# AechPro/rlgym-ppo

Hardware: AMD Instinct MI355X
Metric: ppo_update_samples_per_sec (higher is better)
Workload: dtype f32; 1 GPU; configs[1]: 4096 agents x 128 steps = 524,288-sample buffer, obs 107 f32, 90 discrete actions, 256x3 policy + critic; batch 524,288, minibatch 65,536

## Files before the change

rlgym_ppo_amd/csrc/api.hip:

```cpp
#include "build_id.h"
#include <math.h>
#include <stdarg.h>
#include <string.h>

#include "common.hpp"

namespace rlppo {

static thread_local char g_err[512] = "";

void set_error(const char *fmt, ...) {
    va_list ap;
    va_start(ap, fmt);
    vsnprintf(g_err, sizeof(g_err), fmt, ap);
    va_end(ap);
}

static int64_t padded_width(int64_t d) {
    const int64_t p16 = round_up(d, 16), p64 = round_up(d, 64);
    return (p64 - p16) * 10 >= p64 ? p16 : p64;
}
static int64_t padded_out(int64_t d) {
    if (d <= 32) return 32;
    if (d <= 64) return 64;
// ... 583 lines not shown
        RLPPO_HIP(hipEventCreateWithFlags(&b.ev_join[s], hipEventDisableTiming));
        RLPPO_HIP(hipEventCreateWithFlags(&b.ev_slot[s], hipEventDisableTiming));
        RLPPO_HIP(hipEventCreateWithFlags(&b.ev_mid[s], hipEventDisableTiming));
    }
    return 0;
}
static int order_after(hipStream_t to, hipStream_t from, hipEvent_t ev) {
    RLPPO_HIP(hipEventRecord(ev, from));
    RLPPO_HIP(hipStreamWaitEvent(to, ev, 0));
    return 0;
}

static size_t tn_layer_floats(const NetLayout &net, int l, int64_t mb, int prec) {
    size_t f = tn_partial_floats(net.L[l].out, net.L[l].in, mb);
    if (net.L[l].out == 1) {
        const size_t g = (size_t)cdiv(mb, 64) * (size_t)(net.L[l].pin + 4);
        if (g > f) f = g;
    }
    if (prec == 1 && l == net.n_layers - 1) {
        const size_t g = thin_dw_ws_floats(net.L[l].out, net.L[l].pin, mb);
        if (g > f) f = g;
    }
    return (f + 3) / 4 * 4;
}
static size_t tn_ws_floats(const NetLayout &net, int64_t mb, int prec) {
    size_t m = 0;
    for (int l = 0; l < net.n_layers; ++l) {
        const size_t f = tn_layer_floats(net, l, mb, prec);
        m = f > m ? f : m;
    }
    return m;
}
static int g_group_dw = 1;
struct DwList {
    TnProduct p[2 * RLPPO_MAX_LAYERS];
    int n = 0;
    void add(const LayerLayout &L, const float *dY, const RowSource &X, float *grad) {
        TnProduct &q = p[n++];
        q.dY = dY; q.ldy = L.pout; q.ny_valid = L.pout; q.X = X.x; q.ldx = X.ld; q.kx_valid = L.pin;
        q.dW = grad + L.off_flat_w; q.db = grad + L.off_flat_b; q.out = L.out; q.in = L.in;
        q.rowtab = X.rowtab; q.src_rows = X.src_rows;
    }
};
static bool dw_is_gemv(const NetLayout &net, int l) { return l == net.n_layers - 1 && l > 0 && gemv_head_ok(net.L[l].out, net.L[l].pin); }
static size_t tn_region_floats(const NetLayout &pol, const NetLayout &val, int64_t mb, int prec) {
    const size_t chains = tn_ws_floats(pol, mb, prec) + tn_ws_floats(val, mb, prec);
    int outs[2 * RLPPO_MAX_LAYERS], ins[2 * RLPPO_MAX_LAYERS], n = 0;
    for (const NetLayout *net : {&pol, &val})
        for (int l = 0; l < net->n_layers; ++l)
            if (!dw_is_gemv(*net, l)) {
                outs[n] = net->L[l].out;
                ins[n++] = net->L[l].in;
            }
    const size_t group = tn_group_floats(outs, ins, n, mb);
    return chains > group ? chains : group;
}

struct NetWs {
    float *act[RLPPO_MAX_LAYERS] = {};
    float *dx[RLPPO_MAX_LAYERS] = {};
    unsigned long long *bits[RLPPO_MAX_LAYERS] = {};
    unsigned short *actb[RLPPO_MAX_LAYERS] = {};
    unsigned short *dxb[RLPPO_MAX_LAYERS] = {};
    float *tn = nullptr;
};
struct WsPlan {
    NetWs pol, val;
    size_t tn_floats = 0;
    float *states = nullptr;
    float *g_old = nullptr, *g_adv = nullptr, *g_tgt = nullptr, *g_act = nullptr;
    unsigned *rowtab = nullptr;
    unsigned short *states_b = nullptr;
};
constexpr size_t BITS_PAD_RESERVE = 2, B16_PAD_RESERVE = 4;
static size_t plan_workspace(const NetLayout &pol, const NetLayout &val, int64_t mb, int prec, void *base, WsPlan *w) {
    const uintptr_t addr = reinterpret_cast<uintptr_t>(base);
    const size_t rows = (size_t)mb;
    size_t off = 0, slack = 0;
    auto take = [&](size_t floats) {
        off += floats;
        return reinterpret_cast<float *>(addr + (off - floats) * sizeof(float));
    };
    auto align = [&](size_t floats, size_t reserve) {
        const size_t pad = (floats - (addr / sizeof(float) + off) % floats) % floats;
        off += pad;
        slack += reserve - pad;
    };
    const NetLayout *nets[2] = {&pol, &val};
    NetWs *ws[2] = {&w->pol, &w->val};
    for (int i = 0; i < 2; ++i)
        for (int l = 0; l < nets[i]->n_layers; ++l) ws[i]->act[l] = take(rows * nets[i]->L[l].pout);
    const size_t m = max_pout(pol) > max_pout(val) ? max_pout(pol) : max_pout(val);
    for (int i = 0; i < 2; ++i)
        for (int l = 0; l + 1 < nets[i]->n_layers; ++l) ws[i]->dx[l] = take(rows * m);
    w->tn_floats = tn_region_floats(pol, val, mb, prec);
    w->pol.tn = take(w->tn_floats);
    w->val.tn = w->pol.tn + tn_ws_floats(pol, mb, prec);
    align(2, BITS_PAD_RESERVE);
    for (int i = 0; i < 2; ++i)
        for (int l = 0; l + 1 < nets[i]->n_layers; ++l) {
            const size_t f = nt_bits_floats(mb, nets[i]->L[l].pout);
            ws[i]->bits[l] = f ? reinterpret_cast<unsigned long long *>(take(f)) : nullptr;
        }
    w->states = take(rows * pol.L[0].pin);
    w->g_old = take(rows);
    w->g_adv = take(rows);
    w->g_tgt = take(rows);
// ... 688 lines not shown
        if (xl.fwd[l] >= 0) {
            rc = launch_pack_split((hipStream_t)stream, packed + L.off_w, L.pin, L.pout, L.pin, pl + xl.fwd[l]);
            if (rc) return rc;
        }
        if (xl.dx[l] >= 0) {
            rc = launch_pack_split((hipStream_t)stream, packed + L.off_wt, L.pout, L.pin, L.pout, pl + xl.dx[l]);
            if (rc) return rc;
        }
    }
    return 0;
}
int rlppo_dbg_pack_x3(void *stream, const float *S, int64_t ld, int32_t R, int32_t C, void *planes) {
    return launch_pack_split((hipStream_t)stream, S, ld, R, C, reinterpret_cast<unsigned short *>(planes));
}
int rlppo_dbg_gemm_nt_x3(void *stream, const float *A, int64_t lda, const void *planes, const float *bias, float *C, int64_t ldc, int64_t M,
                         int32_t N, int32_t K, int32_t mode, void *bits) {
    return launch_gemm_nt_split((hipStream_t)stream, A, lda, reinterpret_cast<const unsigned short *>(planes), bias, C, ldc, M, N, K, mode,
                                reinterpret_cast<unsigned long long *>(bits));
}
static int64_t g_selection_epoch = 0;
int rlppo_set_update_precision(int32_t mode) {
    RLPPO_CHECK_ARG(mode >= 0 && mode <= 2, "set_update_precision: mode %d (0 = fp32, 1 = bf16 mixed precision, 2 = split-bf16 products)", mode);
    g_update_bf16 = mode;
    ++g_selection_epoch;
    return 0;
}
int rlppo_get_update_precision(void) { return g_update_bf16; }
int rlppo_set_inference_precision(int32_t mode) {
    RLPPO_CHECK_ARG(mode == 0 || mode == 1, "set_inference_precision: mode %d (0 = fp32, 1 = bf16 operands)", mode);
    set_infer_bf16(mode);
    ++g_selection_epoch;
    return 0;
}
int rlppo_dbg_set(int32_t key, int32_t value) {
    ++g_selection_epoch;
    switch (key) {
        case 1: set_gae_algo(value); return 0;
        case 4: g_two_streams = value; return 0;
        case 21: set_gae_spin_limit(value); return 0;
        case 22: set_gae_oversubscribe(value); return 0;
        case 34: set_fused_spin_limit(value); return 0;
        case 35: set_fused_test_hold(value); return 0;
        case 36: set_split_persistent(value); return 0;
        case 23: set_b16_wide_tiles(value); return 0;
        case 24: set_exp_fast_transform(value); return 0;
        case 26: g_fused_gather = value; return 0;
        case 27: g_fused_act = value; return 0;
        case 29: g_paired = value; return 0;
        case 31: g_head_order = value; return 0;
        case 32: g_fold_vhead = value; return 0;
        case 33: set_pair_interleave(value); return 0;
        case 37: g_group_dw = value; return 0;
        case 38: set_tn_group_budget(value); return 0;
        case 40: set_nt_skinny(value); return 0;
        case 41: g_window_mode = value; return 0;
        default: break;
    }
    set_error("dbg_set: unknown key %d", key);
    return RLPPO_ERR_ARG;
}
int64_t rlppo_selection_epoch(void) { return g_selection_epoch; }
const int64_t *rlppo_selection_epoch_ptr(void) { return &g_selection_epoch; }
int64_t rlppo_dbg_counter(int32_t key) {
    switch (key) {
        case 0: return g_cnt_fused_act;
        case 1: return g_cnt_act_chain;
        case 2: return g_cnt_pass;
        case 3: return g_cnt_paired_pass;
        case 4: return g_cnt_gather_fused_pass;
        case 5: return g_cnt_group_dw;
        default: return -1;
    }
}
size_t rlppo_dbg_gemm_nt_bits_bytes(int64_t M, int32_t N) { return nt_bits_floats(M, N) * sizeof(float); }
int rlppo_dbg_gemm_nt_bits(void *stream, const float *A, int64_t lda, const float *B, int64_t ldb, const float *bias, float *C,
                           int64_t ldc, int64_t M, int32_t N, int32_t K, int32_t epilogue, void *bits) {
    const int rc = launch_gemm_nt_bits((hipStream_t)stream, A, lda, B, ldb, bias, C, ldc, M, N, K, epilogue,
                                       reinterpret_cast<unsigned long long *>(bits));
    if (rc == -1) {
        set_error("dbg_gemm_nt_bits: the bitmask form does not apply to this call");
        return RLPPO_ERR_ARG;
    }
    return rc;
}
int rlppo_dbg_gemm_nt(void *stream, const float *A, int64_t lda, const float *B, int64_t ldb, const float *bias,
                      const float *mask_src, int64_t ld_mask, float *C, int64_t ldc, int64_t M, int32_t N, int32_t K,
                      int32_t epilogue) {
    return launch_gemm_nt((hipStream_t)stream, A, lda, B, ldb, bias, mask_src, ld_mask, C, ldc, M, N, K, epilogue);
}
int rlppo_dbg_gemm_nt_b16(void *stream, const void *A, int64_t lda, const void *W, int64_t ldw, const float *bias, float *C,
                          int64_t ldc, void *Cb, int64_t ldcb, int64_t M, int32_t N, int32_t K, int32_t epilogue, int32_t hidden,
                          void *bits) {
    return launch_gemm_nt_b16((hipStream_t)stream, reinterpret_cast<const unsigned short *>(A), lda,
                              reinterpret_cast<const unsigned short *>(W), ldw, bias, C, ldc, reinterpret_cast<unsigned short *>(Cb),
                              ldcb, M, N, K, epilogue, hidden, reinterpret_cast<unsigned long long *>(bits));
}
int rlppo_dbg_gemm_tn_b16(void *stream, const void *dY, int64_t ldy, const void *X, int64_t ldx, float *dW, float *db, int32_t pout,
                          int32_t pin, int32_t out, int32_t in, int64_t M, void *ws, size_t ws_bytes) {
    return launch_gemm_tn_b16((hipStream_t)stream, reinterpret_cast<const unsigned short *>(dY), ldy,
                              reinterpret_cast<const unsigned short *>(X), ldx, dW, db, pout, pin, out, in, M, (float *)ws,
                              ws_bytes / sizeof(float));
}
size_t rlppo_dbg_thin_head_workspace_bytes(int32_t out, int32_t kp, int64_t M) { return thin_dw_ws_floats(out, kp, M) * sizeof(float); }
int rlppo_dbg_thin_head_b16(void *stream, const float *dY, int64_t ldy, int32_t out, const float *W, int64_t ldw, const void *bits,
                            const void *hb, int64_t ldh, void *dxb, float *dW, float *db, int32_t in, int32_t kp, int64_t M, void *ws,
                            size_t ws_bytes) {
// ... 39 lines not shown
```

rlgym_ppo_amd/csrc/common.hpp:

```cpp
#pragma once
#include <hip/hip_runtime.h>
#include <stdint.h>
#include <stdio.h>

#include <atomic>

#include "../../include/rlppo.h"

namespace rlppo {

void set_error(const char *fmt, ...);

#define RLPPO_CHECK_ARG(cond, ...)                \
    do {                                          \
        if (!(cond)) {                            \
            rlppo::set_error(__VA_ARGS__);        \
            return RLPPO_ERR_ARG;                 \
        }                                         \
    } while (0)

#define RLPPO_HIP(expr)                                                                         \
    do {                                                                                        \
        hipError_t e_ = (expr);                                                                 \
        if (e_ != hipSuccess) {                                                                 \
// ... 54 lines not shown
};

int make_layout(const int32_t *dims, int32_t n_layers, NetLayout *out);

enum Epilogue { EPI_BIAS = 0, EPI_BIAS_RELU = 1, EPI_BIAS_TANH = 2, EPI_MASK = 3 };

int launch_gemm_nt(hipStream_t st, const float *A, int64_t lda, const float *B, int64_t ldb, const float *bias,
                   const float *mask_src, int64_t ld_mask, float *C, int64_t ldc, int64_t M, int N, int K, int epi,
                   int bf16_operands = 0);
size_t nt_bits_floats(int64_t M, int N);
struct NtAlt {
    const float *A = nullptr, *B = nullptr, *bias = nullptr;
    float *C = nullptr;
    unsigned long long *bits = nullptr;
    int interleave = 0;
};
struct NtDot {
    const float *w = nullptr, *b = nullptr;
    float *out = nullptr;
};
struct TnPair {
    const float *dY = nullptr, *X = nullptr;
    float *dW = nullptr, *db = nullptr, *ws = nullptr;
};
int launch_gemm_nt_bits(hipStream_t st, const float *A, int64_t lda, const float *B, int64_t ldb, const float *bias, float *C,
                        int64_t ldc, int64_t M, int N, int K, int epi, unsigned long long *bits, const unsigned *rowtab = nullptr,
                        int64_t src_rows = 0, const NtAlt *alt = nullptr, const NtDot *dot = nullptr );
bool nt_gather_ok(int64_t lda, int64_t src_rows, int N, int K);
int launch_gemm_nt_bf16(hipStream_t st, const float *A, int64_t lda, const float *B, int64_t ldb, const float *bias, float *C,
                        int64_t ldc, int64_t M, int N, int nb, int K, int epi);
void set_infer_bf16(int v);
void set_pair_interleave(int v);
void set_nt_skinny(int on);
int get_infer_bf16();
size_t tn_partial_floats(int out, int in, int64_t M);
int launch_gemm_tn(hipStream_t st, const float *dY, int64_t ldy, int ny_valid, const float *X, int64_t ldx, int kx_valid,
                   float *dW, float *db, int out, int in, int64_t M, float *ws, size_t ws_floats, const unsigned *rowtab = nullptr,
                   int64_t src_rows = 0, const TnPair *pair = nullptr);
bool tn_gather_ok(int64_t ldx, int64_t src_rows);
struct TnProduct {
    const float *dY = nullptr;
    int64_t ldy = 0;
    int ny_valid = 0;
    const float *X = nullptr;
    int64_t ldx = 0;
    int kx_valid = 0;
    float *dW = nullptr, *db = nullptr;
    int out = 0, in = 0;
    const unsigned *rowtab = nullptr;
    int64_t src_rows = 0;
};
constexpr int TN_GROUP_MAX = 2 * RLPPO_MAX_LAYERS;
size_t tn_group_floats(const int *outs, const int *ins, int n, int64_t M);
int launch_gemm_tn_group(hipStream_t st, const TnProduct *prods, int n, int64_t M, float *ws, size_t ws_floats);
void set_tn_group_budget(int workgroups);

bool nt_b16_ok(int N, int K, bool hidden);
bool nt_split_ok(int N, int K);
void set_split_persistent(int v);
int launch_pack_split(hipStream_t st, const float *S, int64_t ld, int R, int Cc, unsigned short *planes);
int launch_gemm_nt_split(hipStream_t st, const float *A, int64_t lda, const unsigned short *planes, const float *bias, float *C, int64_t ldc,
                         int64_t M, int N, int K, int mode, unsigned long long *bits);
int launch_gemm_nt_b16(hipStream_t st, const unsigned short *A, int64_t lda, const unsigned short *B, int64_t ldb, const float *bias,
                       float *C, int64_t ldc, unsigned short *Cb, int64_t ldcb, int64_t M, int N, int K, int epi, int mode,
                       unsigned long long *bits);
void set_b16_wide_tiles(int on);
bool tn_b16_ok(int pout, int pin);
int launch_gemm_tn_b16(hipStream_t st, const unsigned short *dY, int64_t ldy, const unsigned short *X, int64_t ldx, float *dW,
                       float *db, int pout, int pin, int out, int in, int64_t M, float *ws, size_t ws_floats);

void set_exp_fast_transform(int on);

bool gemv_head_ok(int out, int kp);
int launch_gemv_fwd(hipStream_t st, const float *x, int64_t ldx, const float *w, const float *b, float *y, int64_t ldy, int64_t n, int kp, int pout);
int launch_gemv_fwd_b16(hipStream_t st, const unsigned short *x, int64_t ldx, const float *w, const float *b, float *y, int64_t ldy,
                        int64_t n, int kp, int pout);
bool thin_head_ok(int out, int kp);
size_t thin_dw_ws_floats(int out, int kp, int64_t n);
int launch_thin_dx_b16(hipStream_t st, const float *dy, int64_t ldy, int out, const float *w, int64_t ldw,
                       const unsigned long long *bits, unsigned short *dxb, int64_t ldc, int kp, int64_t n);
int launch_thin_dw_b16(hipStream_t st, const float *dy, int64_t ldy, const unsigned short *xb, int64_t ldx, float *dw, float *db,
                       int out, int in, int kp, int64_t n, float *ws, size_t ws_floats);
int launch_gemv_dx(hipStream_t st, const float *dy, int64_t ldy, const float *w, const float *mask, int64_t ldm, float *dx, int64_t ldc, int kp, int64_t n);
int launch_gemv_dx_bits(hipStream_t st, const float *dy, int64_t ldy, const float *w, const unsigned long long *bits, float *dx,
                        int64_t ldc, int kp, int64_t n);
int launch_gemv_dw(hipStream_t st, const float *dy, int64_t ldy, const float *x, int64_t ldx, float *dw, float *db, int in, int kp, int64_t n,
                   float *ws = nullptr, size_t ws_floats = 0);

struct LossCfg {
    float clip, clip_lo, clip_hi, ent_coef, mb_ratio, inv_mb;
    float var_m, var_b;
    const float *adv_norm = nullptr;
    float vclip = 0.f;
    double *kl_slots = nullptr;
    const unsigned *stop_word = nullptr;
};
__host__ __device__ __forceinline__ int64_t ring_row(int64_t i, int64_t base, int64_t cap) {
    const int64_t r = i + base;
    return r >= cap ? r - cap : r;
}
int launch_discrete_sample_logits(hipStream_t, const float *, int64_t, int64_t, int, const float *, int64_t *, float *, float *,
                                  const unsigned *mask = nullptr, int mask_words = 0);
int launch_discrete_probs(hipStream_t st, const float *logits, int64_t ld, int64_t n, int A, int clamp, float *probs,
                          int64_t ld_p, int64_t *flat_argmax, const unsigned *mask = nullptr, int mask_words = 0);
struct MaskRows {
    const unsigned *mask = nullptr;
    int W = 0;
    const int64_t *idx = nullptr;
// ... 88 lines not shown
```

rlgym_ppo_amd/csrc/gemm.hip:

```cpp
#include "gemm_detail.hpp"

namespace rlppo {

template <int NB, int EPI, int BKT, bool BITS = false, bool GATHER = false>
__global__ __launch_bounds__(256, BKT == 16 ? 4 : 2) void gemm_nt_dma_kernel(const float *__restrict__ A, unsigned lda_b,
                                                                              const float *__restrict__ B, unsigned ldb_b,
                                                                              const float *__restrict__ bias,
                                                                              const float *__restrict__ mask_src,
                                                                              unsigned ldm_b, float *__restrict__ C,
                                                                              unsigned ldc_b, int64_t M, int K,
                                                                              unsigned long long *__restrict__ bits = nullptr,
                                                                              const unsigned *__restrict__ rowtab = nullptr,
                                                                              unsigned src_rows = 0, NtAlt alt = NtAlt{},
                                                                              NtDot dot = NtDot{}, NtDot dot_alt = NtDot{}) {
    constexpr int BN = NB * 16;
    constexpr int CPR = BKT / 4;
    constexpr int RPW = 64 / CPR;
    constexpr int RPP = 4 * RPW;
    constexpr int A_IT = SBM / RPP, B_IT = BN / RPP;
    constexpr int B_REM = BN % RPP;
    static_assert(B_REM % RPW == 0, "the ragged staging pass must be whole wave instructions");
    __shared__ __attribute__((aligned(16))) float lds[2 * SBM * BKT + 2 * BN * BKT];
    float *As = lds;
    float *Bs = lds + 2 * SBM * BKT;
// ... 431 lines not shown

int launch_gemm_nt(hipStream_t st, const float *A, int64_t lda, const float *B, int64_t ldb, const float *bias,
                   const float *mask_src, int64_t ld_mask, float *C, int64_t ldc, int64_t M, int N, int K, int epi,
                   int bf16_operands) {
    if (M <= 0) return 0;
    RLPPO_CHECK_ARG(K > 0 && K % 16 == 0, "gemm_nt: K=%d must be a positive multiple of 16", K);
    RLPPO_CHECK_ARG(lda % 4 == 0 && ldb % 4 == 0 && ldc % 4 == 0 && lda >= K && ldb >= K && ldc >= N,
                    "gemm_nt: leading dimensions lda=%ld ldb=%ld ldc=%ld incompatible with K=%d N=%d", (long)lda,
                    (long)ldb, (long)ldc, K, N);
    RLPPO_CHECK_ARG(epi != EPI_MASK || (mask_src && ld_mask >= N && ld_mask % 4 == 0), "gemm_nt: mask operand missing");
    RLPPO_CHECK_ARG(epi == EPI_MASK || bias, "gemm_nt: bias operand missing");
    int nb;
    if (N % 128 == 0) nb = 8;
    else if (N == 96) nb = 6;
    else if (N == 64) nb = 4;
    else if (N == 32) nb = 2;
    else {
        set_error("gemm_nt: N=%d is not a padded output width", N);
        return RLPPO_ERR_ARG;
    }
    const int64_t lim = (int64_t)1 << 31;
    RLPPO_CHECK_ARG(129 * lda * 4 < lim && 129 * ldb * 4 < lim && 129 * ldc * 4 < lim && 129 * ld_mask * 4 < lim,
                    "gemm_nt: a leading dimension is too wide for 32-bit tile offsets");
    if (bf16_operands && epi != EPI_MASK && K % 32 == 0) return launch_gemm_nt_bf16(st, A, lda, B, ldb, bias, C, ldc, M, N, nb, K, epi);
    if (g_nt_skinny && M <= SK_MAX_ROWS && epi != EPI_MASK && !bf16_operands) return launch_gemm_nt_skinny(st, A, lda, B, ldb, bias, C, ldc, M, N, K, epi);
    dim3 grid((unsigned)cdiv(M, SBM), (unsigned)(N / (nb * 16)));
    const unsigned la = (unsigned)(lda * 4), lb = (unsigned)(ldb * 4), lc = (unsigned)(ldc * 4), lm = (unsigned)(ld_mask * 4);
    switch (nb) {
        case 8: return launch_nt_1<8>(st, grid, epi, A, la, B, lb, bias, mask_src, lm, C, lc, M, K);
        case 6: return launch_nt_1<6>(st, grid, epi, A, la, B, lb, bias, mask_src, lm, C, lc, M, K);
        case 4: return launch_nt_1<4>(st, grid, epi, A, la, B, lb, bias, mask_src, lm, C, lc, M, K);
        default: return launch_nt_1<2>(st, grid, epi, A, la, B, lb, bias, mask_src, lm, C, lc, M, K);
    }
}

namespace {
constexpr int TM = 32;
constexpr unsigned OOR = 0x80000000u;
}

struct TnGeom {
    int ni, nj, wn;
    __host__ __device__ int bnt() const { return wn * ni * 16; }
    __host__ __device__ int bkx() const { return (4 / wn) * nj * 16; }
    __host__ __device__ int tile_floats() const { return ni * nj * 1024; }
};
static TnGeom tn_geometry(int out, int in) {
    if (in > 96 && in <= 112) return TnGeom{2, 7, 4};
    if (out > 64 && out <= 96) return TnGeom{3, 4, 2};
    return TnGeom{4, 4, 2};
}

constexpr int TN_LDS_FLOATS = 2 * 2 * 32 * 128;
template <int TMT, int NI, int NJ, int WN, bool GATHER>
__device__ __forceinline__ void tn_tile(float *lds, const float *__restrict__ dY, unsigned ldy_b, int ny_valid,
                                        const float *__restrict__ X, unsigned ldx_b, int kx_valid, bool with_db, int out, int64_t M,
                                        int rows_per_wg, float *__restrict__ partial, const unsigned *__restrict__ rowtab,
                                        unsigned src_rows, int bx, int by, int bz, int tiles_x, int tiles_y, int splits_z) {
    constexpr int WK = 4 / WN;
    constexpr int BNT = WN * NI * 16, BKX = WK * NJ * 16, TILE_F = NI * NJ * 1024;
    constexpr int PPW = TMT / 8;
    static_assert(2 * 2 * TMT * 128 <= TN_LDS_FLOATS && 8 * 128 <= TN_LDS_FLOATS, "stage buffers");
    float *Ys = lds;
    float *Xs = lds + 2 * TMT * 128;

    const int tid = threadIdx.x;
    const int lane = tid & 63, wave = tid >> 6;
    const int wave_u = __builtin_amdgcn_readfirstlane(wave);
    const int r16 = lane & 15, q = lane >> 4;
    const int wn = wave / WK, wk = wave % WK;
    const int n0 = bx * BNT, k0 = by * BKX;
    const int64_t mbeg = (int64_t)bz * rows_per_wg;
    const int rows = (int)((M - mbeg) < rows_per_wg ? (M - mbeg) : rows_per_wg);
    const int steps = (rows + TMT - 1) / TMT;
    const int rem = rows - (steps - 1) * TMT;
    const int ny_here = (ny_valid - n0) < BNT ? (ny_valid - n0) : BNT;
    const int kx_here = (kx_valid - k0) < BKX ? (kx_valid - k0) : BKX;

    const __amdgpu_buffer_rsrc_t y_rs = make_rsrc(reinterpret_cast<const char *>(dY) + mbeg * ldy_b + (int64_t)n0 * 4,
                                                  (unsigned)(rows - 1) * ldy_b + (unsigned)ny_here * 4);
    const __amdgpu_buffer_rsrc_t x_rs =
        GATHER ? __builtin_amdgcn_make_buffer_rsrc(const_cast<float *>(X), (short)ldx_b, src_rows, 0x00020000)
               : make_rsrc(reinterpret_cast<const char *>(X) + mbeg * ldx_b + (int64_t)k0 * 4,
                           (unsigned)(rows - 1) * ldx_b + (unsigned)kx_here * 4);
    const int row_l = 2 * wave + (lane >> 5);
    const int lch = (lane & 31) ^ ((row_l & 3) << 2);
    const bool x_col = lch * 4 < kx_here;
    const unsigned y_off = (lch * 4 < ny_here) ? (unsigned)row_l * ldy_b + lch * 16 : OOR;
    const unsigned x_off = GATHER ? (unsigned)(k0 * 4 + lch * 16) : (x_col ? (unsigned)row_l * ldx_b + lch * 16 : OOR);
    const unsigned y_row8 = 8u * ldy_b, x_row8 = 8u * ldx_b, y_stage = TMT * ldy_b, x_stage = TMT * ldx_b;
    unsigned x_row[4];
    static_assert(PPW <= 4, "x_row");
    const __amdgpu_buffer_rsrc_t t_rs = make_rsrc(GATHER ? rowtab + mbeg : nullptr, GATHER ? (unsigned)rows * 4 : 0u);
    auto load_rows = [&](int stage) {
        if (GATHER) {
#pragma unroll
            for (int i = 0; i < PPW; ++i)
                x_row[i] = __builtin_amdgcn_raw_buffer_load_b32(t_rs, (unsigned)row_l * 4, (unsigned)(stage * TMT + 8 * i) * 4, 0);
        }
    };

    auto issue_stage = [&](int buf, int stage) {
        float *Yd = Ys + (buf * TMT + 2 * wave_u) * 128, *Xd = Xs + (buf * TMT + 2 * wave_u) * 128;
#pragma unroll
        for (int i = 0; i < PPW; ++i) {
            __builtin_amdgcn_raw_ptr_buffer_load_lds(y_rs, Yd + 8 * i * 128, 16, y_off, (unsigned)stage * y_stage + i * y_row8, 0, 0);
            if (GATHER) {
                if (x_col) __builtin_amdgcn_struct_ptr_buffer_load_lds(x_rs, Xd + 8 * i * 128, 16, x_row[i], x_off, 0, 0, 0);
            } else {
                __builtin_amdgcn_raw_ptr_buffer_load_lds(x_rs, Xd + 8 * i * 128, 16, x_off, (unsigned)stage * x_stage + i * x_row8, 0, 0);
            }
        }
    };
    const int zr = tid >> 5, zc = (tid & 31) * 4;
    auto clear_tail = [&](int buf) {
        const f32x4 z = f32x4{0.f, 0.f, 0.f, 0.f};
        for (int r = rem + zr; r < TMT; r += 8) {
            *reinterpret_cast<f32x4 *>(&Ys[(buf * TMT + r) * 128 + zc]) = z;
            *reinterpret_cast<f32x4 *>(&Xs[(buf * TMT + r) * 128 + zc]) = z;
        }
    };

    f32x4 acc[NI][NJ], acc2[NI][NJ];
#pragma unroll
    for (int i = 0; i < NI; ++i)
#pragma unroll
        for (int j = 0; j < NJ; ++j) acc[i][j] = acc2[i][j] = f32x4{0.f, 0.f, 0.f, 0.f};
    f32x4 bs4 = f32x4{0.f, 0.f, 0.f, 0.f};
    const bool want_db = with_db && by == 0;

    load_rows(0);
    if (GATHER) asm volatile("s_waitcnt vmcnt(0)" ::: "memory");
    issue_stage(0, 0);
    if (steps > 1) load_rows(1);
    asm volatile("s_waitcnt vmcnt(0)" ::: "memory");
    if (steps == 1 && rem < TMT) clear_tail(0);
    __syncthreads();
    int fy[NI], fx[NJ];
#pragma unroll
    for (int i = 0; i < NI; ++i) {
        const int g = wn * NI + i;
        fy[i] = q * 128 + (((g & ~3) | ((g & 3) ^ q)) << 4) + r16;
    }
#pragma unroll
    for (int j = 0; j < NJ; ++j) {
        const int g = wk * NJ + j;
        fx[j] = q * 128 + (((g & ~3) | ((g & 3) ^ q)) << 4) + r16;
    }
    const int db_off = zr * 128 + zc;
    for (int st = 0; st < steps; ++st) {
        const int cur = st & 1;
        const bool more = (st + 1) < steps;
        if (more) {
            issue_stage(cur ^ 1, st + 1);
            if ((st + 2) < steps) load_rows(st + 2);
        }
        const float *Yc = Ys + cur * TMT * 128;
        const float *Xc = Xs + cur * TMT * 128;
        if (want_db) {
#pragma unroll
            for (int i = 0; i < PPW; ++i) bs4 += *reinterpret_cast<const f32x4 *>(&Yc[db_off + 8 * i * 128]);
        }
#pragma unroll
        for (int c = 0; c < TMT / 16; ++c) {
#pragma unroll
            for (int s = 0; s < 4; ++s) {
                const int m = c * 16 + s * 4;
                float fa[NI], fb[NJ];
#pragma unroll
                for (int i = 0; i < NI; ++i) fa[i] = Yc[m * 128 + fy[i]];
#pragma unroll
                for (int j = 0; j < NJ; ++j) fb[j] = Xc[m * 128 + fx[j]];
#pragma unroll
                for (int i = 0; i < NI; ++i)
#pragma unroll
                    for (int j = 0; j < NJ; ++j) {
                        if (c & 1) acc2[i][j] = MFMA16(fa[i], fb[j], acc2[i][j]);
                        else acc[i][j] = MFMA16(fa[i], fb[j], acc[i][j]);
                    }
            }
        }
        __builtin_amdgcn_sched_barrier(0);
        asm volatile("s_waitcnt vmcnt(0)" ::: "memory");
        if (more && (st + 2) == steps && rem < TMT) clear_tail(cur ^ 1);
        __syncthreads();
    }

    if (want_db) {
        float *red = lds;
        const int lcol = ((tid & 31) ^ ((zr & 3) << 2)) * 4;
        *reinterpret_cast<f32x4 *>(&red[zr * 128 + lcol]) = bs4;
        __syncthreads();
        if (tid < BNT && (n0 + tid) < out) {
            float sum = 0.f;
#pragma unroll
            for (int r = 0; r < 8; ++r) sum += red[r * 128 + tid];
            partial[(size_t)splits_z * tiles_y * tiles_x * TILE_F + ((size_t)bz * tiles_x + bx) * 128 + tid] = sum;
        }
    }
#pragma unroll
    for (int i = 0; i < NI; ++i)
#pragma unroll
        for (int j = 0; j < NJ; ++j) acc[i][j] += acc2[i][j];
    __builtin_amdgcn_sched_barrier(0);
    {
        const size_t tile_id = (size_t)bz * (tiles_x * tiles_y) + (size_t)by * tiles_x + bx;
        const __amdgpu_buffer_rsrc_t p_rs = make_rsrc(partial + tile_id * TILE_F, TILE_F * 4);
#pragma unroll
        for (int i = 0; i < NI; ++i)
#pragma unroll
            for (int j = 0; j < NJ; ++j) stb(p_rs, (unsigned)tid * 16, (unsigned)(i * NJ + j) * 4096, acc[i][j]);
    }
}

template <int TMT, int NI, int NJ, int WN, bool GATHER>
__global__ __launch_bounds__(256, 2) void gemm_tn_dma_kernel(const float *__restrict__ dY, unsigned ldy_b,
                                                                              int ny_valid, const float *__restrict__ X,
                                                                              unsigned ldx_b, int kx_valid,
                                                                              bool with_db, int out, int in, int64_t M,
                                                                              int rows_per_wg, float *__restrict__ partial,
                                                                              const unsigned *__restrict__ rowtab,
                                                                              unsigned src_rows, TnAlt alt) {
    __shared__ __attribute__((aligned(16))) float lds[TN_LDS_FLOATS];
    const int splits_z = alt.dY ? gridDim.z / 2 : gridDim.z;
    int zloc = blockIdx.z;
    bool second = alt.dY && !alt.interleave && zloc >= splits_z;
    if (second) zloc -= splits_z;
    int il_tile = -1, il_split = 0;
    if (alt.dY && alt.interleave) {
        const int T = gridDim.x * gridDim.y;
        const int id = (blockIdx.z * gridDim.y + blockIdx.y) * gridDim.x + blockIdx.x, g = id % (16 * T);
        int t2 = g >> 3;
        second = t2 >= T;
        if (second) t2 -= T;
        il_tile = t2;
        il_split = (id / (16 * T)) * 8 + (g & 7);
    }
    if (second) {
        dY = alt.dY;
        if (!GATHER) X = alt.X;
        partial = alt.partial;
    }
    int bx = blockIdx.x, by = blockIdx.y, bz = zloc;
    {
        const int T = gridDim.x * gridDim.y;
        if (il_tile >= 0) {
            bz = il_split;
            bx = il_tile % gridDim.x;
            by = il_tile / gridDim.x;
        } else if ((splits_z & 7) == 0 && T > 1) {
            const int id = (zloc * gridDim.y + blockIdx.y) * gridDim.x + blockIdx.x, g = id % (8 * T);
            const int tile = g >> 3;
            bz = (id / (8 * T)) * 8 + (g & 7);
            bx = tile % gridDim.x;
            by = tile / gridDim.x;
        }
    }
    tn_tile<TMT, NI, NJ, WN, GATHER>(lds, dY, ldy_b, ny_valid, X, ldx_b, kx_valid, with_db, out, M, rows_per_wg, partial, rowtab, src_rows,
                                     bx, by, bz, (int)gridDim.x, (int)gridDim.y, splits_z);
}


__device__ __forceinline__ void tn_reduce_tile(const float *__restrict__ partial, int splits, int tiles_x, int tiles,
                                               float *__restrict__ dW, float *__restrict__ db, int out, int in, TnGeom geo, int tile,
                                               int bxi, int nbx, float (*red)[64][4], float *dbh) {
    const int e64 = threadIdx.x & 63, sl = threadIdx.x >> 6;
    const int elem4 = bxi * 64 + e64;
    const int tile4 = geo.tile_floats() / 4;
    const f32x4 *base = reinterpret_cast<const f32x4 *>(partial) + (size_t)tile * tile4 + elem4;
    const size_t stride = (size_t)tiles * tile4;
    f32x4 acc = f32x4{0.f, 0.f, 0.f, 0.f};
    int sp = sl;
    for (; sp + 28 < splits; sp += 32) {
        f32x4 v[8];
#pragma unroll
        for (int u = 0; u < 8; ++u) v[u] = __builtin_nontemporal_load(base + (size_t)(sp + 4 * u) * stride);
#pragma unroll
        for (int u = 0; u < 8; ++u) acc += v[u];
    }
    for (; sp + 12 < splits; sp += 16) {
        f32x4 v[4];
#pragma unroll
        for (int u = 0; u < 4; ++u) v[u] = __builtin_nontemporal_load(base + (size_t)(sp + 4 * u) * stride);
#pragma unroll
        for (int u = 0; u < 4; ++u) acc += v[u];
    }
    for (; sp < splits; sp += 4) acc += __builtin_nontemporal_load(base + (size_t)sp * stride);
    if (sl > 0) *reinterpret_cast<f32x4 *>(&red[sl - 1][e64][0]) = acc;
    const int bnt = geo.bnt(), bkx = geo.bkx();
    const bool db_block = db && bxi == nbx - 1 && tile < tiles_x;
    float sdb = 0.f;
    if (db_block) {
        const int c = threadIdx.x & 127, half = threadIdx.x >> 7;
        const float *pdb = partial + (size_t)splits * tiles * geo.tile_floats() + (size_t)tile * 128 + c;
        const size_t dstride = (size_t)tiles_x * 128;
        const int s_lo = half ? (splits + 1) / 2 : 0, s_hi = half ? splits : (splits + 1) / 2;
        float a16[16];
#pragma unroll
        for (int u = 0; u < 16; ++u) a16[u] = 0.f;
        int s2 = s_lo;
        if (c < bnt) {
            for (; s2 + 15 < s_hi; s2 += 16) {
                float v[16];
#pragma unroll
                for (int u = 0; u < 16; ++u) v[u] = pdb[(size_t)(s2 + u) * dstride];
#pragma unroll
                for (int u = 0; u < 16; ++u) a16[u] += v[u];
            }
            for (int u = 0; s2 < s_hi; ++s2, ++u) a16[u] += pdb[(size_t)s2 * dstride];
        }
#pragma unroll
// ... 63 lines not shown
                   float *dW, float *db, int out, int in, int64_t M, float *ws, size_t ws_floats, const unsigned *rowtab,
                   int64_t src_rows, const TnPair *pair) {
    if (M <= 0) return 0;
    RLPPO_CHECK_ARG(ny_valid % 4 == 0 && kx_valid % 4 == 0 && ldy % 4 == 0 && ldx % 4 == 0 && ny_valid <= ldy &&
                        kx_valid <= ldx && out <= ny_valid && in <= kx_valid,
                    "gemm_tn: bad shapes ny=%d kx=%d ldy=%ld ldx=%ld out=%d in=%d", ny_valid, kx_valid, (long)ldy,
                    (long)ldx, out, in);
    if (!ws || ws_floats < tn_partial_floats(out, in, M)) {
        set_error("gemm_tn: workspace %zu < %zu floats", ws ? ws_floats : (size_t)0, tn_partial_floats(out, in, M));
        return RLPPO_ERR_WORKSPACE;
    }
    const TnGeom g = tn_geometry(out, in);
    const int tiles_x = (int)cdiv(out, g.bnt()), tiles_y = (int)cdiv(in, g.bkx());
    const int rows_per_wg = (int)tn_rows_for((int64_t)tiles_x * tiles_y, M);
    const int splits = (int)cdiv(M, rows_per_wg);
    const int64_t lim = (int64_t)1 << 30;
    RLPPO_CHECK_ARG((rows_per_wg + TM) * ldy * 4 < lim && (rowtab || (rows_per_wg + TM) * ldx * 4 < lim),
                    "gemm_tn: a leading dimension is too wide for 32-bit tile offsets");
    RLPPO_CHECK_ARG(!rowtab || tn_gather_ok(ldx, src_rows), "gemm_tn (gathered rows): unsupported row stride %ld", (long)ldx);
    RLPPO_CHECK_ARG(!pair || (pair->dY && (rowtab || pair->X) && pair->dW && pair->ws && (pair->db != nullptr) == (db != nullptr)),
                    "gemm_tn: incomplete second operand set");
    dim3 grid((unsigned)tiles_x, (unsigned)tiles_y, (unsigned)(pair ? 2 * splits : splits));
    TnAlt alt{};
    if (pair) alt = TnAlt{pair->dY, pair->X, pair->ws, (g_pair_interleave && splits % 8 == 0) ? 1 : 0};
#define TN(NI_, NJ_, WN_, G_)                                                                                              \
    hipLaunchKernelGGL((gemm_tn_dma_kernel<TM, NI_, NJ_, WN_, G_>), grid, dim3(256), 0, st, dY, (unsigned)(ldy * 4), ny_valid, X, \
                       (unsigned)(ldx * 4), kx_valid, db != nullptr, out, in, M, rows_per_wg, ws, rowtab, (unsigned)src_rows, alt)
    if (g.nj == 7) {
        if (rowtab) TN(2, 7, 4, true); else TN(2, 7, 4, false);
    } else if (g.ni == 3) {
        RLPPO_CHECK_ARG(!rowtab, "gemm_tn (gathered rows): the 96-row tile has no gathered form");
        TN(3, 4, 2, false);
    } else {
        if (rowtab) TN(4, 4, 2, true); else TN(4, 4, 2, false);
    }
#undef TN
    RLPPO_LAUNCH_CHECK();
    TnRedAlt ralt{};
    if (pair) ralt = TnRedAlt{pair->ws, pair->dW, pair->db};
    return launch_tn_reduce(st, ws, splits, tiles_x, tiles_y, dW, db, out, in, g.ni, g.nj, g.wn, pair ? &ralt : nullptr);
}
int launch_tn_reduce(hipStream_t st, const float *partial, int splits, int tiles_x, int tiles_y, float *dW, float *db, int out, int in,
                     int ni, int nj, int wn, const TnRedAlt *alt) {
    hipLaunchKernelGGL(tn_reduce_kernel, dim3((unsigned)(ni * nj * 4), (unsigned)(tiles_x * tiles_y), alt ? 2u : 1u), dim3(256), 0, st,
                       partial, splits, tiles_x, tiles_x * tiles_y, dW, db, out, in, TnGeom{ni, nj, wn}, alt ? *alt : TnRedAlt{});
    RLPPO_LAUNCH_CHECK();
    return 0;
}
struct TnWork {
    const float *dY, *X;
    float *partial;
    const unsigned *rowtab;
    unsigned ldy_b, ldx_b, src_rows;
    int ny_valid, kx_valid, out, rows_per_wg, splits, tiles_x, tiles_y, with_db, geom, wg_begin;
};
struct TnGroupArgs {
    int n;
    int64_t M;
    TnWork w[TN_GROUP_MAX];
};
__global__ __launch_bounds__(256, 2) void gemm_tn_group_kernel(TnGroupArgs g) {
    __shared__ __attribute__((aligned(16))) float lds[TN_LDS_FLOATS];
    const int id = blockIdx.x;
    int p = 0;
    for (int i = 1; i < g.n; ++i)
        if (id >= g.w[i].wg_begin) p = i;
    const TnWork &w = g.w[p];
    const int loc = id - w.wg_begin, T = w.tiles_x * w.tiles_y, S8 = w.splits & ~7;
    int tile, bz;
    if (loc < S8 * T) {
        const int gq = loc % (8 * T);
        tile = gq >> 3;
        bz = (loc / (8 * T)) * 8 + (gq & 7);
    } else {
        const int r = loc - S8 * T, R = w.splits - S8;
        if (R <= 0 || r >= R * T) return;
        tile = r / R;
        bz = S8 + r % R;
    }
    const int bx = tile % w.tiles_x, by = tile / w.tiles_x;
#define TN_ITEM(NI_, NJ_, WN_, G_)                                                                                                     \
    tn_tile<TM, NI_, NJ_, WN_, G_>(lds, w.dY, w.ldy_b, w.ny_valid, w.X, w.ldx_b, w.kx_valid, w.with_db != 0, w.out, g.M, w.rows_per_wg, \
                                   w.partial, w.rowtab, w.src_rows, bx, by, bz, w.tiles_x, w.tiles_y, w.splits)
    switch (w.geom) {
        case 0: TN_ITEM(4, 4, 2, false); break;
        case 1: TN_ITEM(4, 4, 2, true); break;
        case 2: TN_ITEM(3, 4, 2, false); break;
        case 3: TN_ITEM(2, 7, 4, false); break;
        default: TN_ITEM(2, 7, 4, true); break;
    }
#undef TN_ITEM
}

struct TnRedWork {
    const float *partial;
    float *dW, *db;
    int splits, tiles_x, tiles, out, in, tile_begin;
    TnGeom geo;
};
struct TnRedGroupArgs {
    int n;
    TnRedWork w[TN_GROUP_MAX];
};
__global__ __launch_bounds__(256) void tn_reduce_group_kernel(TnRedGroupArgs g) {
    __shared__ __attribute__((aligned(16))) float red[3][64][4];
    __shared__ float dbh[128];
    const int t = blockIdx.y;
    int p = 0;
    for (int i = 1; i < g.n; ++i)
        if (t >= g.w[i].tile_begin) p = i;
    const TnRedWork &w = g.w[p];
    const int nbx = w.geo.ni * w.geo.nj * 4;
    if ((int)blockIdx.x >= nbx) return;
    tn_reduce_tile(w.partial, w.splits, w.tiles_x, w.tiles, w.dW, w.db, w.out, w.in, w.geo, t - w.tile_begin, (int)blockIdx.x, nbx, red, dbh);
}

static int g_tn_group_budget = 0;
constexpr int TN_MAX_CHAIN = 8192;
void set_tn_group_budget(int v) { g_tn_group_budget = v; }
struct TnPlanItem {
    TnGeom g;
    int tiles_x, tiles_y, splits, rows_per_wg, wg_begin;
    size_t partial_off, floats;
};
static int tn_group_plan(const int *outs, const int *ins, int n, int64_t M, int budget, TnPlanItem *it, int *total_wgs, size_t *total_floats) {
    for (int p = 0; p < n; ++p) {
        it[p].g = tn_geometry(outs[p], ins[p]);
        it[p].tiles_x = (int)cdiv(outs[p], it[p].g.bnt());
        it[p].tiles_y = (int)cdiv(ins[p], it[p].g.bkx());
    }
    const int64_t max_splits = cdiv(M, 32);
    auto fill = [&](double t) {
        int64_t wgs = 0;
        for (int p = 0; p < n; ++p) {
            const int blocks = it[p].g.ni * it[p].g.nj;
            int64_t rows = (int64_t)(t / blocks);
            rows = round_up(rows < 32 ? 32 : rows, 32);
            if (g_tn_group_budget <= 0 && rows > TN_MAX_CHAIN) rows = TN_MAX_CHAIN;
            int64_t sp = cdiv(M, rows);
            if (sp > max_splits) sp = max_splits;
            rows = round_up(cdiv(M, sp), 32);
            it[p].rows_per_wg = (int)rows;
            it[p].splits = (int)cdiv(M, rows);
            wgs += round_up((int64_t)it[p].splits * it[p].tiles_x * it[p].tiles_y, 8);
        }
        return wgs;
    };
    for (int rounds = g_tn_group_budget > 0 ? 1 : 2;; ++rounds) {
        const int64_t cap = (int64_t)budget * rounds;
        double lo = 32.0, hi = (double)round_up(M, 32) * 32.0;
        if (fill(lo) <= cap) break;
        for (int i = 0; i < 60; ++i) {
            const double mid = 0.5 * (lo + hi);
            if (fill(mid) > cap) lo = mid; else hi = mid;
        }
        if (fill(hi) <= cap || g_tn_group_budget > 0 || rounds >= 256) break;
    }
    int wg = 0;
    size_t off = 0;
    for (int p = 0; p < n; ++p) {
        it[p].wg_begin = wg;
        wg += (int)round_up((int64_t)it[p].splits * it[p].tiles_x * it[p].tiles_y, 8);
        it[p].partial_off = off;
        it[p].floats = (size_t)it[p].splits * it[p].tiles_x * it[p].tiles_y * (size_t)it[p].g.tile_floats() + (size_t)it[p].splits * it[p].tiles_x * 128;
        off += (it[p].floats + 3) / 4 * 4;
    }
    *total_wgs = wg;
    *total_floats = off;
    return 0;
}
static int tn_group_budget() {
    if (g_tn_group_budget > 0) return g_tn_group_budget;
    int cus = 0;
    if (device_cu_count(&cus) || cus <= 0) cus = 256;
    return 2 * cus;
}
size_t tn_group_floats(const int *outs, const int *ins, int n, int64_t M) {
    if (n <= 0 || M <= 0) return 0;
    size_t total = 0;
    for (int b = 0; b < n; b += TN_GROUP_MAX) {
        TnPlanItem it[TN_GROUP_MAX];
        int wgs = 0;
        size_t f = 0;
        const int m = n - b < TN_GROUP_MAX ? n - b : TN_GROUP_MAX;
        tn_group_plan(outs + b, ins + b, m, M, tn_group_budget(), it, &wgs, &f);
        total = f > total ? f : total;
    }
    return total;
}
int launch_gemm_tn_group(hipStream_t st, const TnProduct *prods, int n, int64_t M, float *ws, size_t ws_floats) {
    if (M <= 0 || n <= 0) return 0;
    for (int b = 0; b < n; b += TN_GROUP_MAX) {
        const int m = n - b < TN_GROUP_MAX ? n - b : TN_GROUP_MAX;
        const TnProduct *pr = prods + b;
        int outs[TN_GROUP_MAX], ins[TN_GROUP_MAX];
        for (int p = 0; p < m; ++p) {
            outs[p] = pr[p].out;
            ins[p] = pr[p].in;
        }
        TnPlanItem it[TN_GROUP_MAX];
        int wgs = 0;
        size_t floats = 0;
        tn_group_plan(outs, ins, m, M, tn_group_budget(), it, &wgs, &floats);
        if (!ws || ws_floats < floats) {
            set_error("gemm_tn_group: workspace %zu < %zu floats", ws ? ws_floats : (size_t)0, floats);
            return RLPPO_ERR_WORKSPACE;
        }
        TnGroupArgs ga{};
        TnRedGroupArgs ra{};
        ga.n = ra.n = m;
        ga.M = M;
        const int64_t lim = (int64_t)1 << 30;
        int tile_begin = 0;
        for (int p = 0; p < m; ++p) {
            const TnProduct &q = pr[p];
            RLPPO_CHECK_ARG(q.dY && q.X && q.dW && q.ny_valid % 4 == 0 && q.kx_valid % 4 == 0 && q.ldy % 4 == 0 && q.ldx % 4 == 0 &&
                                q.ny_valid <= q.ldy && q.kx_valid <= q.ldx && q.out <= q.ny_valid && q.in <= q.kx_valid,
                            "gemm_tn_group: bad shapes (product %d) ny=%d kx=%d ldy=%ld ldx=%ld out=%d in=%d", p, q.ny_valid, q.kx_valid,
                            (long)q.ldy, (long)q.ldx, q.out, q.in);
            RLPPO_CHECK_ARG(((int64_t)it[p].rows_per_wg + TM) * q.ldy * 4 < lim && (q.rowtab || ((int64_t)it[p].rows_per_wg + TM) * q.ldx * 4 < lim),
                            "gemm_tn_group: a leading dimension is too wide for 32-bit tile offsets");
            RLPPO_CHECK_ARG(!q.rowtab || tn_gather_ok(q.ldx, q.src_rows), "gemm_tn_group (gathered rows): unsupported row stride %ld", (long)q.ldx);
            RLPPO_CHECK_ARG(!(q.rowtab && it[p].g.ni == 3), "gemm_tn_group (gathered rows): the 96-row tile has no gathered form");
            TnWork &w = ga.w[p];
            w.dY = q.dY;
            w.X = q.X;
            w.partial = ws + it[p].partial_off;
            w.rowtab = q.rowtab;
            w.ldy_b = (unsigned)(q.ldy * 4);
            w.ldx_b = (unsigned)(q.ldx * 4);
            w.src_rows = (unsigned)q.src_rows;
            w.ny_valid = q.ny_valid;
            w.kx_valid = q.kx_valid;
            w.out = q.out;
            w.rows_per_wg = it[p].rows_per_wg;
            w.splits = it[p].splits;
            w.tiles_x = it[p].tiles_x;
            w.tiles_y = it[p].tiles_y;
            w.with_db = q.db != nullptr;
            w.geom = it[p].g.nj == 7 ? (q.rowtab ? 4 : 3) : it[p].g.ni == 3 ? 2 : (q.rowtab ? 1 : 0);
            w.wg_begin = it[p].wg_begin;
            TnRedWork &r = ra.w[p];
            r.partial = w.partial;
            r.dW = q.dW;
            r.db = q.db;
            r.splits = it[p].splits;
            r.tiles_x = it[p].tiles_x;
            r.tiles = it[p].tiles_x * it[p].tiles_y;
            r.out = q.out;
            r.in = q.in;
            r.tile_begin = tile_begin;
            r.geo = it[p].g;
            tile_begin += r.tiles;
        }
        hipLaunchKernelGGL(gemm_tn_group_kernel, dim3((unsigned)wgs), dim3(256), 0, st, ga);
        RLPPO_LAUNCH_CHECK();
        hipLaunchKernelGGL(tn_reduce_group_kernel, dim3(64u, (unsigned)tile_begin), dim3(256), 0, st, ra);
        RLPPO_LAUNCH_CHECK();
    }
    return 0;
}
}
```

Measured before the change: 64.68 million samples/s.

## Taper split-K row chunks in grouped TN dW GEMM and flush accumulators periodically

The grouped weight-gradient GEMM planner no longer caps row chunks at 8192 by default. It splits each product's row range into a head segment of large chunks and a tail segment of smaller chunks, and the tail workgroups are launched after all head workgroups so the end of the grid is better balanced. The kernel now accumulates into a single accumulator set and folds it into a second set every 512 rows, replacing the alternating dual-accumulator chain. This keeps precision bounded for long chains but adds planner complexity and a larger workspace bound, and the MFMA dependency chain gets longer.

```diff
diff --git a/rlgym_ppo_amd/csrc/api.hip b/rlgym_ppo_amd/csrc/api.hip
--- a/rlgym_ppo_amd/csrc/api.hip
+++ b/rlgym_ppo_amd/csrc/api.hip
@@ -659,7 +659,7 @@
                 outs[n] = net->L[l].out;
                 ins[n++] = net->L[l].in;
             }
-    const size_t group = tn_group_floats(outs, ins, n, mb);
+    const size_t group = tn_group_floats_bound(outs, ins, n, mb);
     return chains > group ? chains : group;
 }
 
@@ -1454,6 +1454,8 @@
         case 33: set_pair_interleave(value); return 0;
         case 37: g_group_dw = value; return 0;
         case 38: set_tn_group_budget(value); return 0;
+        case 42: set_tn_group_taper(value, -1); return 0;
+        case 43: set_tn_group_taper(-1, value); return 0;
         case 40: set_nt_skinny(value); return 0;
         case 41: g_window_mode = value; return 0;
         default: break;
diff --git a/rlgym_ppo_amd/csrc/common.hpp b/rlgym_ppo_amd/csrc/common.hpp
--- a/rlgym_ppo_amd/csrc/common.hpp
+++ b/rlgym_ppo_amd/csrc/common.hpp
@@ -130,8 +130,10 @@
 };
 constexpr int TN_GROUP_MAX = 2 * RLPPO_MAX_LAYERS;
 size_t tn_group_floats(const int *outs, const int *ins, int n, int64_t M);
+size_t tn_group_floats_bound(const int *outs, const int *ins, int n, int64_t M);
 int launch_gemm_tn_group(hipStream_t st, const TnProduct *prods, int n, int64_t M, float *ws, size_t ws_floats);
 void set_tn_group_budget(int workgroups);
+void set_tn_group_taper(int share, int ratio);
 
 bool nt_b16_ok(int N, int K, bool hidden);
 bool nt_split_ok(int N, int K);
diff --git a/rlgym_ppo_amd/csrc/gemm.hip b/rlgym_ppo_amd/csrc/gemm.hip
--- a/rlgym_ppo_amd/csrc/gemm.hip
+++ b/rlgym_ppo_amd/csrc/gemm.hip
@@ -507,10 +507,14 @@
 }
 
 constexpr int TN_LDS_FLOATS = 2 * 2 * 32 * 128;
+#ifndef TN_FLUSH_ROWS
+#define TN_FLUSH_ROWS 512
+#endif
+static_assert(TN_FLUSH_ROWS % 32 == 0 && TN_FLUSH_ROWS >= 32, "a flush falls on a stage boundary");
 template <int TMT, int NI, int NJ, int WN, bool GATHER>
 __device__ __forceinline__ void tn_tile(float *lds, const float *__restrict__ dY, unsigned ldy_b, int ny_valid,
                                         const float *__restrict__ X, unsigned ldx_b, int kx_valid, bool with_db, int out, int64_t M,
-                                        int rows_per_wg, float *__restrict__ partial, const unsigned *__restrict__ rowtab,
+                                        int64_t mbeg, int rows_cap, float *__restrict__ partial, const unsigned *__restrict__ rowtab,
                                         unsigned src_rows, int bx, int by, int bz, int tiles_x, int tiles_y, int splits_z) {
     constexpr int WK = 4 / WN;
     constexpr int BNT = WN * NI * 16, BKX = WK * NJ * 16, TILE_F = NI * NJ * 1024;
@@ -525,8 +529,7 @@
     const int r16 = lane & 15, q = lane >> 4;
     const int wn = wave / WK, wk = wave % WK;
     const int n0 = bx * BNT, k0 = by * BKX;
-    const int64_t mbeg = (int64_t)bz * rows_per_wg;
-    const int rows = (int)((M - mbeg) < rows_per_wg ? (M - mbeg) : rows_per_wg);
+    const int rows = (int)((M - mbeg) < rows_cap ? (M - mbeg) : rows_cap);
     const int steps = (rows + TMT - 1) / TMT;
     const int rem = rows - (steps - 1) * TMT;
     const int ny_here = (ny_valid - n0) < BNT ? (ny_valid - n0) : BNT;
@@ -576,6 +579,8 @@
         }
     };
 
+    constexpr int FLUSH_STAGES = TN_FLUSH_ROWS / TMT;
+    static_assert(TN_FLUSH_ROWS % TMT == 0, "flush interval");
     f32x4 acc[NI][NJ], acc2[NI][NJ];
 #pragma unroll
     for (int i = 0; i < NI; ++i)
@@ -629,13 +634,19 @@
 #pragma unroll
                 for (int i = 0; i < NI; ++i)
 #pragma unroll
-                    for (int j = 0; j < NJ; ++j) {
-                        if (c & 1) acc2[i][j] = MFMA16(fa[i], fb[j], acc2[i][j]);
-                        else acc[i][j] = MFMA16(fa[i], fb[j], acc[i][j]);
-                    }
+                    for (int j = 0; j < NJ; ++j) acc[i][j] = MFMA16(fa[i], fb[j], acc[i][j]);
             }
         }
         __builtin_amdgcn_sched_barrier(0);
+        if ((st + 1) % FLUSH_STAGES == 0) {
+#pragma unroll
+            for (int i = 0; i < NI; ++i)
+#pragma unroll
+                for (int j = 0; j < NJ; ++j) {
+                    acc2[i][j] += acc[i][j];
+                    acc[i][j] = f32x4{0.f, 0.f, 0.f, 0.f};
+                }
+        }
         asm volatile("s_waitcnt vmcnt(0)" ::: "memory");
         if (more && (st + 2) == steps && rem < TMT) clear_tail(cur ^ 1);
         __syncthreads();
@@ -711,7 +722,7 @@
             by = tile / gridDim.x;
         }
     }
-    tn_tile<TMT, NI, NJ, WN, GATHER>(lds, dY, ldy_b, ny_valid, X, ldx_b, kx_valid, with_db, out, M, rows_per_wg, partial, rowtab, src_rows,
+    tn_tile<TMT, NI, NJ, WN, GATHER>(lds, dY, ldy_b, ny_valid, X, ldx_b, kx_valid, with_db, out, M, (int64_t)bz * rows_per_wg, rows_per_wg, partial, rowtab, src_rows,
                                      bx, by, bz, (int)gridDim.x, (int)gridDim.y, splits_z);
 }
 
@@ -881,7 +892,7 @@
     float *partial;
     const unsigned *rowtab;
     unsigned ldy_b, ldx_b, src_rows;
-    int ny_valid, kx_valid, out, rows_per_wg, splits, tiles_x, tiles_y, with_db, geom, wg_begin;
+    int ny_valid, kx_valid, out, rows_a, splits_a, rows_b, splits_b, tiles_x, tiles_y, with_db, geom, wg_a, wg_b;
 };
 struct TnGroupArgs {
     int n;
@@ -891,26 +902,31 @@
 __global__ __launch_bounds__(256, 2) void gemm_tn_group_kernel(TnGroupArgs g) {
     __shared__ __attribute__((aligned(16))) float lds[TN_LDS_FLOATS];
     const int id = blockIdx.x;
+    const bool tail = id >= g.w[0].wg_b;
     int p = 0;
     for (int i = 1; i < g.n; ++i)
-        if (id >= g.w[i].wg_begin) p = i;
+        if (id >= (tail ? g.w[i].wg_b : g.w[i].wg_a)) p = i;
     const TnWork &w = g.w[p];
-    const int loc = id - w.wg_begin, T = w.tiles_x * w.tiles_y, S8 = w.splits & ~7;
+    const int S = tail ? w.splits_b : w.splits_a;
+    const int loc = id - (tail ? w.wg_b : w.wg_a), T = w.tiles_x * w.tiles_y, S8 = S & ~7;
     int tile, bz;
     if (loc < S8 * T) {
         const int gq = loc % (8 * T);
         tile = gq >> 3;
         bz = (loc / (8 * T)) * 8 + (gq & 7);
     } else {
-        const int r = loc - S8 * T, R = w.splits - S8;
+        const int r = loc - S8 * T, R = S - S8;
         if (R <= 0 || r >= R * T) return;
         tile = r / R;
         bz = S8 + r % R;
     }
     const int bx = tile % w.tiles_x, by = tile / w.tiles_x;
-#define TN_ITEM(NI_, NJ_, WN_, G_)                                                                                                     \
-    tn_tile<TM, NI_, NJ_, WN_, G_>(lds, w.dY, w.ldy_b, w.ny_valid, w.X, w.ldx_b, w.kx_valid, w.with_db != 0, w.out, g.M, w.rows_per_wg, \
-                                   w.partial, w.rowtab, w.src_rows, bx, by, bz, w.tiles_x, w.tiles_y, w.splits)
+    const int64_t mbeg = tail ? (int64_t)w.splits_a * w.rows_a + (int64_t)bz * w.rows_b : (int64_t)bz * w.rows_a;
+    const int rows_cap = tail ? w.rows_b : w.rows_a;
+    if (tail) bz += w.splits_a;
+#define TN_ITEM(NI_, NJ_, WN_, G_)                                                                                                  \
+    tn_tile<TM, NI_, NJ_, WN_, G_>(lds, w.dY, w.ldy_b, w.ny_valid, w.X, w.ldx_b, w.kx_valid, w.with_db != 0, w.out, g.M, mbeg, rows_cap, \
+                                   w.partial, w.rowtab, w.src_rows, bx, by, bz, w.tiles_x, w.tiles_y, w.splits_a + w.splits_b)
     switch (w.geom) {
         case 0: TN_ITEM(4, 4, 2, false); break;
         case 1: TN_ITEM(4, 4, 2, true); break;
@@ -945,19 +961,27 @@
 }
 
 static int g_tn_group_budget = 0;
-constexpr int TN_MAX_CHAIN = 8192;
+static int g_tn_taper_share = 50;
+static int g_tn_taper_ratio = 33;
 void set_tn_group_budget(int v) { g_tn_group_budget = v; }
+void set_tn_group_taper(int share, int ratio) {
+    if (share >= 0) g_tn_taper_share = share > 90 ? 90 : share;
+    if (ratio >= 0) g_tn_taper_ratio = ratio < 5 ? 5 : ratio > 100 ? 100 : ratio;
+}
 struct TnPlanItem {
     TnGeom g;
-    int tiles_x, tiles_y, splits, rows_per_wg, wg_begin;
+    int tiles_x, tiles_y, splits_a, rows_a, splits_b, rows_b, wg_a, wg_b;
     size_t partial_off, floats;
+    int splits() const { return splits_a + splits_b; }
 };
-static int tn_group_plan(const int *outs, const int *ins, int n, int64_t M, int budget, TnPlanItem *it, int *total_wgs, size_t *total_floats) {
+static int tn_group_plan(const int *outs, const int *ins, int n, int64_t M, int budget, TnPlanItem *it, int *total_wgs, size_t *total_floats,
+                         int max_rows = 0) {
     for (int p = 0; p < n; ++p) {
         it[p].g = tn_geometry(outs[p], ins[p]);
         it[p].tiles_x = (int)cdiv(outs[p], it[p].g.bnt());
         it[p].tiles_y = (int)cdiv(ins[p], it[p].g.bkx());
     }
+    if (g_tn_group_budget > 0) max_rows = 0;
     const int64_t max_splits = cdiv(M, 32);
     auto fill = [&](double t) {
         int64_t wgs = 0;
@@ -965,13 +989,14 @@
             const int blocks = it[p].g.ni * it[p].g.nj;
             int64_t rows = (int64_t)(t / blocks);
             rows = round_up(rows < 32 ? 32 : rows, 32);
-            if (g_tn_group_budget <= 0 && rows > TN_MAX_CHAIN) rows = TN_MAX_CHAIN;
+            if (max_rows > 0 && rows > max_rows) rows = max_rows;
             int64_t sp = cdiv(M, rows);
             if (sp > max_splits) sp = max_splits;
             rows = round_up(cdiv(M, sp), 32);
-            it[p].rows_per_wg = (int)rows;
-            it[p].splits = (int)cdiv(M, rows);
-            wgs += round_up((int64_t)it[p].splits * it[p].tiles_x * it[p].tiles_y, 8);
+            it[p].rows_a = (int)rows;
+            it[p].splits_a = (int)cdiv(M, rows);
+            it[p].rows_b = it[p].splits_b = 0;
+            wgs += round_up((int64_t)it[p].splits_a * it[p].tiles_x * it[p].tiles_y, 8);
         }
         return wgs;
     };
@@ -983,16 +1008,37 @@
             const double mid = 0.5 * (lo + hi);
             if (fill(mid) > cap) lo = mid; else hi = mid;
         }
-        if (fill(hi) <= cap || g_tn_group_budget > 0 || rounds >= 256) break;
+        if (fill(hi) <= cap || max_rows <= 0 || rounds >= 256) break;
+    }
+    if (max_rows <= 0 && g_tn_group_budget <= 0 && g_tn_taper_share > 0 && g_tn_taper_ratio < 100) {
+        for (int p = 0; p < n; ++p) {
+            TnPlanItem &q = it[p];
+            if (q.splits_a < 4 || q.rows_a < 256) continue;
+            int sb = (q.splits_a * g_tn_taper_share + 50) / 100;
+            sb = sb < 1 ? 1 : sb;
+            const int sa = q.splits_a - sb;
+            const int64_t ra = round_up(cdiv(M * 100, (int64_t)sa * 100 + (int64_t)sb * g_tn_taper_ratio), 32);
+            const int64_t left = M - sa * ra;
+            if (left < 1) continue;
+            const int64_t rb = round_up(cdiv(left, sb), 32);
+            q.splits_a = sa;
+            q.rows_a = (int)ra;
+            q.rows_b = (int)rb;
+            q.splits_b = (int)cdiv(left, rb);
+        }
     }
     int wg = 0;
     size_t off = 0;
     for (int p = 0; p < n; ++p) {
-        it[p].wg_begin = wg;
-        wg += (int)round_up((int64_t)it[p].splits * it[p].tiles_x * it[p].tiles_y, 8);
+        it[p].wg_a = wg;
+        wg += (int)round_up((int64_t)it[p].splits_a * it[p].tiles_x * it[p].tiles_y, 8);
         it[p].partial_off = off;
-        it[p].floats = (size_t)it[p].splits * it[p].tiles_x * it[p].tiles_y * (size_t)it[p].g.tile_floats() + (size_t)it[p].splits * it[p].tiles_x * 128;
+        it[p].floats = (size_t)it[p].splits() * it[p].tiles_x * it[p].tiles_y * (size_t)it[p].g.tile_floats() + (size_t)it[p].splits() * it[p].tiles_x * 128;
         off += (it[p].floats + 3) / 4 * 4;
+    }
+    for (int p = 0; p < n; ++p) {
+        it[p].wg_b = wg;
+        wg += (int)round_up((int64_t)it[p].splits_b * it[p].tiles_x * it[p].tiles_y, 8);
     }
     *total_wgs = wg;
     *total_floats = off;
@@ -1004,7 +1050,7 @@
     if (device_cu_count(&cus) || cus <= 0) cus = 256;
     return 2 * cus;
 }
-size_t tn_group_floats(const int *outs, const int *ins, int n, int64_t M) {
+static size_t tn_group_floats_of(const int *outs, const int *ins, int n, int64_t M, int max_rows) {
     if (n <= 0 || M <= 0) return 0;
     size_t total = 0;
     for (int b = 0; b < n; b += TN_GROUP_MAX) {
@@ -1012,10 +1058,15 @@
         int wgs = 0;
         size_t f = 0;
         const int m = n - b < TN_GROUP_MAX ? n - b : TN_GROUP_MAX;
-        tn_group_plan(outs + b, ins + b, m, M, tn_group_budget(), it, &wgs, &f);
+        tn_group_plan(outs + b, ins + b, m, M, tn_group_budget(), it, &wgs, &f, max_rows);
         total = f > total ? f : total;
     }
     return total;
+}
+size_t tn_group_floats(const int *outs, const int *ins, int n, int64_t M) { return tn_group_floats_of(outs, ins, n, M, 0); }
+size_t tn_group_floats_bound(const int *outs, const int *ins, int n, int64_t M) {
+    const size_t former = tn_group_floats_of(outs, ins, n, M, 8192), now = tn_group_floats_of(outs, ins, n, M, 0);
+    return former > now ? former : now;
 }
 int launch_gemm_tn_group(hipStream_t st, const TnProduct *prods, int n, int64_t M, float *ws, size_t ws_floats) {
     if (M <= 0 || n <= 0) return 0;
@@ -1047,7 +1098,7 @@
                                 q.ny_valid <= q.ldy && q.kx_valid <= q.ldx && q.out <= q.ny_valid && q.in <= q.kx_valid,
                             "gemm_tn_group: bad shapes (product %d) ny=%d kx=%d ldy=%ld ldx=%ld out=%d in=%d", p, q.ny_valid, q.kx_valid,
                             (long)q.ldy, (long)q.ldx, q.out, q.in);
-            RLPPO_CHECK_ARG(((int64_t)it[p].rows_per_wg + TM) * q.ldy * 4 < lim && (q.rowtab || ((int64_t)it[p].rows_per_wg + TM) * q.ldx * 4 < lim),
+            RLPPO_CHECK_ARG(((int64_t)it[p].rows_a + TM) * q.ldy * 4 < lim && (q.rowtab || ((int64_t)it[p].rows_a + TM) * q.ldx * 4 < lim),
                             "gemm_tn_group: a leading dimension is too wide for 32-bit tile offsets");
             RLPPO_CHECK_ARG(!q.rowtab || tn_gather_ok(q.ldx, q.src_rows), "gemm_tn_group (gathered rows): unsupported row stride %ld", (long)q.ldx);
             RLPPO_CHECK_ARG(!(q.rowtab && it[p].g.ni == 3), "gemm_tn_group (gathered rows): the 96-row tile has no gathered form");
@@ -1062,18 +1113,21 @@
             w.ny_valid = q.ny_valid;
             w.kx_valid = q.kx_valid;
             w.out = q.out;
-            w.rows_per_wg = it[p].rows_per_wg;
-            w.splits = it[p].splits;
+            w.rows_a = it[p].rows_a;
+            w.splits_a = it[p].splits_a;
+            w.rows_b = it[p].rows_b;
+            w.splits_b = it[p].splits_b;
             w.tiles_x = it[p].tiles_x;
             w.tiles_y = it[p].tiles_y;
             w.with_db = q.db != nullptr;
             w.geom = it[p].g.nj == 7 ? (q.rowtab ? 4 : 3) : it[p].g.ni == 3 ? 2 : (q.rowtab ? 1 : 0);
-            w.wg_begin = it[p].wg_begin;
+            w.wg_a = it[p].wg_a;
+            w.wg_b = it[p].wg_b;
             TnRedWork &r = ra.w[p];
             r.partial = w.partial;
             r.dW = q.dW;
             r.db = q.db;
-            r.splits = it[p].splits;
+            r.splits = it[p].splits();
             r.tiles_x = it[p].tiles_x;
             r.tiles = it[p].tiles_x * it[p].tiles_y;
             r.out = q.out;
```

Result: slower. 60.08 million samples/s (-7.1%).
